# eigenfoo/littlemcmc

Measured on AMD Instinct MI355X. Metric: leapfrog-steps/sec (all chains), higher is better.
Workload: dtype f64

## Files before the change

### littlemcmc_amd/csrc/lmc_sampler.hpp

```cpp
#pragma once
#include "lmc_rng.hpp"
#include "lmc_targets.hpp"
#include "lmc_team.hpp"

namespace lmc {

constexpr int kStatusBadInitialEnergy = 1;

enum StatF64 : int {
    kSfStepSize = 0,
    kSfStepSizeBar = 1,
    kSfAccept = 2,
    kSfEnergyError = 3,
    kSfEnergy = 4,
    kSfMaxEnergyError = 5,
    kSfModelLogp = 6,
    kNumStatF64 = 7
};
enum StatI32 : int { kSiDepth = 0 , kSiTreeSize = 1 , kNumStatI32 = 2 };
enum StatU8 : int { kSbDiverging = 0, kSbTune = 1, kSbAccepted = 2, kNumStatU8 = 3 };
enum Counter : int { kCtMaxTreedepth = 0, kCtDivsSample = 1, kCtSamplesAfterTune = 2, kCtLeapfrogs = 3, kCtWaveTicks = 4, kNumCounters = 5 };

struct StatRecord {
    double f64[kNumStatF64];
// ... 377 lines not shown
        tm.sync();
        if (tm.wave() == 0) {
            rng_normals(r, d, out, stage);
            if (lane_id() == 0) {
                bcast[0] = static_cast<double>(r.pos);
                bcast[1] = static_cast<double>(r.has_gauss);
                bcast[2] = r.gauss;
            }
        }
        tm.sync();
        r.pos = first_i32(static_cast<int>(bcast[0]));
        r.has_gauss = first_i32(static_cast<int>(bcast[1]));
        r.gauss = first_f64(bcast[2]);
    }
}

template <int NS, class Target, class TeamT>
__device__ __forceinline__ void leapfrog(TeamT& tm, const Target& tgt, const double (&var)[NS], double eps,
                                         double (&q)[NS], double (&p)[NS], double (&g)[NS],
                                         double& energy, double& logp) {
    const double dt = 0.5 * eps;
#pragma unroll
    for (int s = 0; s < NS; ++s) {
        p[s] = p[s] + dt * g[s];
        const double v = var[s] * p[s];
        q[s] = q[s] + eps * v;
    }
    if constexpr (Target::kLanePartial) {
        double lp = tgt.logp_grad_partial(tm, q, g);
        double kin = 0.0;
#pragma unroll
        for (int s = 0; s < NS; ++s) {
            p[s] = p[s] + dt * g[s];
            kin = __builtin_fma(p[s], var[s] * p[s], kin);
        }
        tm.sum2(lp, kin);
        logp = lp;
        energy = 0.5 * kin - logp;
    } else {
        logp = first_f64(tgt.logp_grad(tm, q, g));
        double kin = 0.0;
#pragma unroll
        for (int s = 0; s < NS; ++s) {
            p[s] = p[s] + dt * g[s];
            kin = __builtin_fma(p[s], var[s] * p[s], kin);
        }
        energy = 0.5 * tm.sum(kin) - logp;
    }
}

typedef __attribute__((address_space(3))) double lds_double;
typedef __attribute__((address_space(1))) double glb_double;
template <int NS, class PTR>
__device__ __forceinline__ void vload_as(PTR base, double (&x)[NS]) {
    PTR p = base + LMC_CHAIN_THREAD * NS;
#pragma unroll
    for (int s = 0; s < NS; ++s) x[s] = p[s];
}
template <int NS, class PTR>
__device__ __forceinline__ void vstore_as(PTR base, const double (&x)[NS]) {
    PTR p = base + LMC_CHAIN_THREAD * NS;
#pragma unroll
    for (int s = 0; s < NS; ++s) p[s] = x[s];
}
struct LevelScalars {
    double w, a, pe, plogp;
    __device__ __forceinline__ void put(int j, double w_, double a_, double c, double d) {
        if (lane_id() == j) { w = w_; a = a_; pe = c; plogp = d; }
    }
    __device__ __forceinline__ void get(int j, double& w_, double& a_, double& c, double& d) const {
        w_ = readlane_f64(w, j); a_ = readlane_f64(a, j); c = readlane_f64(pe, j); d = readlane_f64(plogp, j);
    }
};

struct TransitionOut {
    double accept;
    double energy, energy_error, max_energy_error, model_logp;
    int depth;
    int n_leapfrog;
    int diverging;
    int exhausted;
    int accepted;
};

template <class P>
__device__ inline void hmc_transition_any(P& pol, double e0, double logp0, double step_size, double emax, double path_length,
                                          int max_steps, TransitionOut& out) {
    const double plen = first_f64(pol.uniform() * path_length);
    int n_steps = static_cast<int>(plen / step_size);
    n_steps = n_steps < 1 ? 1 : n_steps;
    n_steps = n_steps > max_steps ? max_steps : n_steps;
    typename P::End c;
    pol.start_state(c);
    double energy = e0, logp = logp0;
    for (int i = 0; i < n_steps; ++i) pol.leapfrog(step_size, c, energy, logp);
    bool diverging = !isfinite(energy);
    double de = first_f64(e0 - energy);
    if (isnan(de)) de = -__builtin_inf();
    if (fabs(de) > emax) diverging = true;
    const double accept = first_f64(fmin(1.0, exp_uniform(de)));
    bool accepted = false;
    if (!diverging) {
        const double u = pol.uniform();
        if (!(u >= accept)) { accepted = true; pol.accept_state(c); }
    }
    out.accept = accept;
    out.energy = energy;
    out.energy_error = de;
    out.max_energy_error = plen;
    out.model_logp = logp;
    out.depth = n_steps;
    out.n_leapfrog = n_steps;
    out.diverging = diverging;
    out.exhausted = 0;
    out.accepted = accepted;
}

template <int NS, class Target, class TeamT>
struct FusedHmcPolicy {
    static constexpr int kNS = NS;
    struct End { double q[NS], p[NS], g[NS]; };
    TeamT& tm; const Target& tgt; const double (&var)[NS]; RngState& rng;
    double (&q)[NS]; const double (&p0)[NS]; const double (&g0)[NS];
    UniformWindow win;
    __device__ __forceinline__ double uniform() { return team_uniform(tm, rng, win); }
    __device__ __forceinline__ void start_state(End& c) const { vcopy(c.q, q); vcopy(c.p, p0); vcopy(c.g, g0); }
    __device__ __forceinline__ void leapfrog(double eps, End& c, double& energy, double& logp) {
        lmc::leapfrog<NS>(tm, tgt, var, eps, c.q, c.p, c.g, energy, logp);
    }
    __device__ __forceinline__ void accept_state(const End& c) { vcopy(q, c.q); }
};
template <int NS, class Target, class TeamT>
__device__ inline void hmc_transition(TeamT& tm, const Target& tgt, const double (&var)[NS], RngState& rng,
                                      double (&q)[NS], const double (&p0)[NS], const double (&g0)[NS],
                                      double e0, double logp0, double step_size, double emax,
                                      double path_length, int max_steps, TransitionOut& out) {
    FusedHmcPolicy<NS, Target, TeamT> pol{tm, tgt, var, rng, q, p0, g0, UniformWindow{0.0, 0, 0}};
    hmc_transition_any(pol, e0, logp0, step_size, emax, path_length, max_steps, out);
}

#ifndef LMC_EXP_LANES_SLOAD
#define LMC_EXP_LANES_SLOAD 2
#endif
constexpr int kRedValues = 6;
constexpr int kExpTableDoubles = 32;
constexpr int kLevelScalDoubles = 96;
#ifndef LMC_PAIR_COLD_LDS
#define LMC_PAIR_COLD_LDS 3
#endif
enum ColdSlot : int { kColdAold = 0, kColdPsum = 1, kColdOp = 2, kColdOq = 3, kColdOg = 4, kNumCold = 5 };
constexpr int kNumColdSlots = kNumCold;

constexpr int run_leaf_group(int ns, int w) { return (w == 1 && ns <= 2) ? 4 : 2; }
template <int NS, int W = 1, int PL = 0, int G = 2>
struct PairLds {
    static_assert(G == 2 || (G == 4 && W == 1), "leaf quads exist for the one-wave kernels");
    static constexpr int DP = 64 * NS * W;
    static constexpr int kRedRows = G == 4 ? 8 : kRedValues;
    static constexpr int kRedWave = 64 * kRedRows;
    static constexpr int kRedSize = (2 * DP > W * kRedWave) ? 2 * DP : W * kRedWave;
    static constexpr int kExp = kRedSize;
    static constexpr int kXsum = kExp + kExpTableDoubles;
    static constexpr int kXsumSize = W > 1 ? 2 * 8 * W : 0;
    static constexpr int kScal = kXsum + kXsumSize;
    static constexpr int kCold = kScal + W * kLevelScalDoubles;
    static_assert(PL == 0 || W == 1, "the deep-tree plan exists for one-wave kernels");
    static constexpr int kColdLds = PL == 1 ? (NS >= 4 ? 0 : (LMC_PAIR_COLD_LDS < 1 ? LMC_PAIR_COLD_LDS : 1))
                                            : (W >= 8 ? (LMC_PAIR_COLD_LDS < 2 ? LMC_PAIR_COLD_LDS : 2) : LMC_PAIR_COLD_LDS);
    static constexpr int kQStage = (G == 4 && (NS >= 2 || PL == 0)) ? 2 : 0;
    static constexpr int kL1 = kCold + kColdLds * DP;
    static constexpr int kL2 = kL1 + (G == 4 ? kQStage : 3) * DP;
    static constexpr int kMinDoubles = kL2;
    static constexpr int kGlbLevels = (kNumCold - kColdLds) * DP;
    __host__ __device__ static constexpr int total_doubles(int nlds) { return kL2 + (nlds > 1 ? (nlds - 1) * 4 * DP : 0); }
};
#ifdef LMC_EXPERIMENTAL_SHAPES
#define LMC_PAIR_SHAPES(X) X(1, 1) X(2, 1) X(4, 1) X(4, 2) X(4, 4) X(2, 8) X(2, 2) X(1, 4)
#else
#define LMC_PAIR_SHAPES(X) X(1, 1) X(2, 1) X(4, 1) X(4, 2) X(4, 4)
#endif
constexpr int pair_min_doubles(int ns, int w, int plan = 0, int g = 2) {
#define X(NSV, WV) if (ns == NSV && w == WV) {                                                                               \
        if (g == 4 && run_leaf_group(NSV, WV) == 4)                                                                          \
            return plan == 1 ? PairLds<NSV, 1, 1, 4>::kMinDoubles : PairLds<NSV, 1, 0, 4>::kMinDoubles;                      \
        return (plan == 1 && WV == 1) ? PairLds<NSV, 1, 1>::kMinDoubles : PairLds<NSV, WV, 0>::kMinDoubles; }
    LMC_PAIR_SHAPES(X)
#undef X
    return 1 << 30;
}
constexpr int pair_total_doubles(int ns, int w, int nlds, int plan = 0, int g = 2) {
#define X(NSV, WV) if (ns == NSV && w == WV) {                                                                               \
        if (g == 4 && run_leaf_group(NSV, WV) == 4)                                                                          \
            return plan == 1 ? PairLds<NSV, 1, 1, 4>::total_doubles(nlds) : PairLds<NSV, 1, 0, 4>::total_doubles(nlds);      \
        return (plan == 1 && WV == 1) ? PairLds<NSV, 1, 1>::total_doubles(nlds) : PairLds<NSV, WV, 0>::total_doubles(nlds); }
    LMC_PAIR_SHAPES(X)
#undef X
    return 1 << 30;
}

struct PairCtx {
    double* lds;
    double* glb;
    int nlds;
    int red_lane;
    int wave_red;
    int wave_scal;
    int wave;
    int xpar;
};

template <int NS, int W = 1, int PL = 0, int G = 2>
__device__ __forceinline__ void red_put(const PairCtx& cx, int v, double x) {
    if constexpr (W == 1) ((lds_double*)cx.lds)[v * 64 + lane_id()] = x;
    else ((lds_double*)cx.lds)[v * 64 + lane_id() + cx.wave_red] = x;
}
template <int NS, int W = 1, int PL = 0, int G = 2>
__device__ __forceinline__ double red_gather(PairCtx& cx) {
    typedef double d2 __attribute__((ext_vector_type(2)));
    typedef __attribute__((address_space(3))) d2 lds_d2;
    asm volatile("" ::: "memory");
    unsigned r0 = static_cast<unsigned>(cx.red_lane);
    asm volatile("" : "+v"(r0));
    lds_double* L = (lds_double*)cx.lds;
    const d2 a = *(const lds_d2*)(size_t)(r0), b = *(const lds_d2*)(size_t)(r0 ^ 16u);
    const d2 c = *(const lds_d2*)(size_t)(r0 ^ 32u), d = *(const lds_d2*)(size_t)(r0 ^ 48u);
    asm volatile("" ::: "memory");
    double s = ((a.x + a.y) + (b.x + b.y)) + ((c.x + c.y) + (d.x + d.y));
    s += dpp_f64<0x111>(s);
    s += dpp_f64<0x112>(s);
    s += dpp_f64<0x114>(s);
    if constexpr (W > 1) {
        const int lane = lane_id();
        lds_double* xs = L + (PairLds<NS, W, PL, G>::kXsum + cx.xpar * (8 * W)) + (lane >> 3) * W;
        if ((lane & 7) == 7) xs[cx.wave] = s;
        __syncthreads();
        double t = xs[0];
#pragma unroll
        for (int w = 1; w < W; ++w) t += xs[w];
        s = t;
        cx.xpar ^= 1;
    }
    return s;
}
__device__ __forceinline__ int red_lane_init(int rows = kRedValues) {
    const int lane = lane_id();
    const int row = lane < 8 * rows ? lane : 0;
    return row * 8 + 2 * ((lane >> 2) & 3);
}
__device__ __forceinline__ bool red_any_nonpositive(double s, int k0, int n) {
    const unsigned long long m = ballot64(s <= 0.0);
    unsigned long long sel = 0ull;
    for (int k = k0; k < k0 + n; ++k) sel |= 1ull << (8 * k + 7);
    return (m & sel) != 0ull;
}

__constant__ double kExpLanesConst[8] = {46.166241308446828,
                                         2.16608493865351192654e-02,
                                         5.96317165397058656256e-12,
                                         1.0 / 720.0, 1.0 / 120.0, 1.0 / 24.0, 1.0 / 6.0, 0.0};
struct ExpLanesConst { double inv, hi, lo, c6, c5, c4, c3; };
__device__ __forceinline__ ExpLanesConst exp_lanes_const() {
    ExpLanesConst c;
#if LMC_EXP_LANES_SLOAD == 2
    typedef const __attribute__((address_space(4))) double cst_double;
    cst_double* p = (cst_double*)kExpLanesConst;
    asm volatile("" : "+s"(p));
    c.inv = p[0]; c.hi = p[1]; c.lo = p[2]; c.c6 = p[3]; c.c5 = p[4]; c.c4 = p[5]; c.c3 = p[6];
#elif LMC_EXP_LANES_SLOAD == 1
    c.inv = kExpLanesConst[0]; c.hi = kExpLanesConst[1]; c.lo = kExpLanesConst[2];
    c.c6 = kExpLanesConst[3]; c.c5 = kExpLanesConst[4]; c.c4 = kExpLanesConst[5]; c.c3 = kExpLanesConst[6];
#else
    c.inv = LMC_SC(46.166241308446828); c.hi = LMC_SC(2.16608493865351192654e-02); c.lo = LMC_SC(5.96317165397058656256e-12);
    c.c6 = LMC_SC(1.0 / 720.0); c.c5 = LMC_SC(1.0 / 120.0); c.c4 = LMC_SC(1.0 / 24.0); c.c3 = LMC_SC(1.0 / 6.0);
#endif
    return c;
}
template <int NS, int W = 1, int PL = 0, int G = 2>
__device__ __forceinline__ double exp_lanes(const PairCtx& cx, const ExpLanesConst& c, double x) {
    const double kf = rint(x * c.inv);
    double r = __builtin_fma(-kf, c.hi, x);
    r = __builtin_fma(-kf, c.lo, r);
    const int ki = static_cast<int>(kf);
    const double t = ((const lds_double*)cx.lds)[PairLds<NS, W, PL, G>::kExp + (ki & 31)];
    double p = fma_sgpr_addend(r, c.c6, c.c5);
    p = fma_sgpr_addend(p, r, c.c4);
    p = fma_sgpr_addend(p, r, c.c3);
    p = __builtin_fma(p, r, 0.5);
    p = __builtin_fma(p, r, 1.0);
    p = __builtin_fma(p, r, 1.0);
    return ldexp(p * t, ki >> 5);
}

template <int NS, int W, int PL, int G, int SLOT>
__device__ __forceinline__ void cold_load(const PairCtx& cx, double (&x)[NS]) {
    using L = PairLds<NS, W, PL, G>;
    if constexpr (SLOT < L::kColdLds) vload_as<NS>((lds_double*)cx.lds + (L::kCold + SLOT * L::DP), x);
    else vload_as<NS>((glb_double*)cx.glb + (SLOT - L::kColdLds) * L::DP, x);
}
template <int NS, int W, int PL, int G, int SLOT>
__device__ __forceinline__ void cold_store(const PairCtx& cx, const double (&x)[NS]) {
    using L = PairLds<NS, W, PL, G>;
    if constexpr (SLOT < L::kColdLds) vstore_as<NS>((lds_double*)cx.lds + (L::kCold + SLOT * L::DP), x);
    else vstore_as<NS>((glb_double*)cx.glb + (SLOT - L::kColdLds) * L::DP, x);
}
template <int NS, int W = 1, int PL = 0, int G = 2>
__device__ __forceinline__ void level1_load(const PairCtx& cx, double (&lp)[NS], double (&rp)[NS], double (&ps)[NS]) {
// ... 212 lines not shown
        int qsrc = -1;
        auto prop_q = [&](double (&t)[NS]) {
            if (qsrc == -1) vcopy(t, cq);
            else if (qsrc == -2) vcopy(t, eq);
            else if (G == 4 && qsrc < -2) {
                if constexpr (PairLds<NS, W, PL, G>::kQStage > 0)
                    vload_as<NS>((lds_double*)cx.lds + (PairLds<NS, W, PL, G>::kL1 + (qsrc == -3 ? PairLds<NS, W, PL, G>::DP : 0)), t);
                else if (qsrc == -3) vcopy(t, q1r);
                else vcopy(t, q0r);
            } else level_load_q<NS, W, PL, G>(cx, qsrc, t);
        };
        int elane = 15;
        double en_last = 0.0, lp_last = 0.0;
        const int D = depth;
        if (D == 0) {
            double v[NS], kinp, lp, en, ev;
            leapfrog_partial<NS>(tm, tgt, var, eps, cq, cp, cg, v, kinp, lp);
            red_put<NS, W, PL, G>(cx, 0, kinp); red_put<NS, W, PL, G>(cx, 1, lp);
            const double s0 = red_gather<NS, W, PL, G>(cx);
            if (leaf_scalars(s0, 1, en, ev) == 1) {
                tw = readlane_f64(ev, 15); ta = readlane_f64(ev, 14);
                en_last = en; lp_last = s0;
                vcopy(tps, cp);
            }
        } else if (G == 2 || D == 1) {
            const int n_pairs = 1 << (D - 1);
            for (int k = 0; k < n_pairs; ++k) {
                double v[NS], kinA, lpA, kinB, lpB;
                leapfrog_partial<NS>(tm, tgt, var, eps, cq, cp, cg, v, kinA, lpA);
                red_put<NS, W, PL, G>(cx, 0, kinA); red_put<NS, W, PL, G>(cx, 1, lpA);
                vcopy(eq, cq); vcopy(ep, cp);
                leapfrog_partial<NS>(tm, tgt, var, eps, cq, cp, cg, v, kinB, lpB);
                red_put<NS, W, PL, G>(cx, 2, kinB); red_put<NS, W, PL, G>(cx, 3, lpB);
#pragma unroll
                for (int s = 0; s < NS; ++s) tps[s] = ep[s] + cp[s];
                red_put<NS, W, PL, G>(cx, 4, pdot_v<NS>(tps, var, ep));
                red_put<NS, W, PL, G>(cx, 5, pdot<NS>(tps, v));
                const double s0 = red_gather<NS, W, PL, G>(cx);
                const int m = __builtin_ctz(~static_cast<unsigned>(k) | (1u << (D - 1)));
                double en, ev;
                if (leaf_scalars(s0, 2, en, ev) != 2) break;
                {
                    const double wA = readlane_f64(ev, 15), aA = readlane_f64(ev, 14);
                    const double wB = readlane_f64(ev, 31), aB = readlane_f64(ev, 30);
                    const bool turn = red_any_nonpositive(s0, 4, 2);
                    const double wsum = wA + wB;
                    const bool take_b = uniform_true(team_uniform(tm, rng, win) * wsum < wB);
                    qsrc = take_b ? -1 : -2;
                    elane = take_b ? 31 : 15;
                    en_last = en; lp_last = s0;
                    tw = wsum; ta = aA + aB;
                    if (turn) { turning = true; break; }
                }
                if constexpr (G == 2) {
                if (m >= 1) {
                    double alp[NS], arp[NS], aps[NS];
                    double aw, aa;
                    level1_load<NS, W, PL, G>(cx, alp, arp, aps);
                    level_scal_get_wa<NS, W, PL, G>(cx, 1, aw, aa);
                    const double sj = cascade_dots<NS, W, PL, G>(cx, var, alp, arp, aps, ep, tps, v);
                    const bool turn = red_any_nonpositive(sj, 0, 6);
                    const double wsum = aw + tw;
                    const bool take_b = uniform_true(team_uniform(tm, rng, win) * wsum < tw);
                    if (!take_b) qsrc = 1;
                    tw = wsum; ta = aa + ta;
                    if (turn) { turning = true; break; }
                }
                for (int j = 2; j <= m; ++j) {
                    double blp[NS], brp[NS], bps[NS], tl[NS];
                    levelN_load<NS, W, PL, G>(cx, j, 0, blp); levelN_load<NS, W, PL, G>(cx, j, 1, brp); levelN_load<NS, W, PL, G>(cx, j, 2, bps);
                    level_load_lp<NS, W, PL, G>(cx, j - 1, tl);
                    double bw, ba;
                    level_scal_get_wa<NS, W, PL, G>(cx, j, bw, ba);
                    const double sj = cascade_dots<NS, W, PL, G>(cx, var, blp, brp, bps, tl, tps, v);
                    const bool turn = red_any_nonpositive(sj, 0, 6);
                    const double wsum = bw + tw;
                    const bool take_b = uniform_true(team_uniform(tm, rng, win) * wsum < tw);
                    if (!take_b) qsrc = j;
                    tw = wsum; ta = ba + ta;
                    if (turn) { turning = true; break; }
                }
                if (turning) break;
                if (k + 1 < n_pairs) {
                    double tl[NS], tqv[NS];
                    if (m == 0) vcopy(tl, ep); else level_load_lp<NS, W, PL, G>(cx, m, tl);
                    if (qsrc == -1) vcopy(tqv, cq);
                    else if (qsrc == -2) vcopy(tqv, eq);
                    else level_load_q<NS, W, PL, G>(cx, qsrc, tqv);
#ifndef LMC_PARK_REORDER_MIN_NS
#define LMC_PARK_REORDER_MIN_NS 4
#endif
                    constexpr bool kParkReorder = NS >= LMC_PARK_REORDER_MIN_NS;
                    if constexpr (kParkReorder) level_scal_park<NS, W, PL, G>(cx, m + 1, tw, ta, qsrc, elane, en_last, lp_last);
                    if (m == 0) {
                        level1_store<NS, W, PL, G>(cx, tl, cp, tqv);
                    } else {
                        if constexpr (kParkReorder) {
#pragma unroll
                            for (int s = 0; s < NS; ++s) asm volatile("" : "+v"(tl[s]), "+v"(tqv[s]));
                        }
                        levelN_store<NS, W, PL, G>(cx, m + 1, 0, tl); levelN_store<NS, W, PL, G>(cx, m + 1, 1, cp);
                        levelN_store<NS, W, PL, G>(cx, m + 1, 2, tps); levelN_store<NS, W, PL, G>(cx, m + 1, 3, tqv);
                    }
                    if constexpr (!kParkReorder) level_scal_park<NS, W, PL, G>(cx, m + 1, tw, ta, qsrc, elane, en_last, lp_last);
                }
                }
            }
        } else if constexpr (G == 4) {
            using L = PairLds<NS, W, PL, G>;
            lds_double* const qst = (lds_double*)cx.lds + L::kL1;
            const int n_quads = 1 << (D - 2);
            for (int k = 0; k < n_quads; ++k) {
                static_assert(NS <= 2, "leaf quads: the left end of a depth-2 subtree waits in two rows of the reduction buffer");
                double v[NS], kin, lpl, a0[NS], a1[NS];
                leapfrog_partial<NS>(tm, tgt, var, eps, cq, cp, cg, v, kin, lpl);
                red_put<NS, W, PL, G>(cx, 0, kin); red_put<NS, W, PL, G>(cx, 1, lpl);
                if constexpr (L::kQStage > 0) vstore_as<NS>(qst, cq); else vcopy(q0r, cq);
                vcopy(a0, cp);
                leapfrog_partial<NS>(tm, tgt, var, eps, cq, cp, cg, v, kin, lpl);
                red_put<NS, W, PL, G>(cx, 2, kin); red_put<NS, W, PL, G>(cx, 3, lpl);
                if constexpr (L::kQStage > 0) vstore_as<NS>(qst + L::DP, cq); else vcopy(q1r, cq);
                vcopy(a1, cp);
                leapfrog_partial<NS>(tm, tgt, var, eps, cq, cp, cg, v, kin, lpl);
                red_put<NS, W, PL, G>(cx, 4, kin); red_put<NS, W, PL, G>(cx, 5, lpl);
                vcopy(eq, cq); vcopy(ep, cp);
                leapfrog_partial<NS>(tm, tgt, var, eps, cq, cp, cg, v, kin, lpl);
                red_put<NS, W, PL, G>(cx, 6, kin); red_put<NS, W, PL, G>(cx, 7, lpl);
                const double s0 = red_gather<NS, W, PL, G>(cx);
                double ta01[NS], va1[NS];
#pragma unroll
                for (int s = 0; s < NS; ++s) { ta01[s] = a0[s] + a1[s]; va1[s] = var[s] * a1[s]; tps[s] = ep[s] + cp[s]; }
                red_put<NS, W, PL, G>(cx, 0, pdot_v<NS>(ta01, var, a0));
                red_put<NS, W, PL, G>(cx, 1, pdot<NS>(ta01, va1));
                red_put<NS, W, PL, G>(cx, 2, pdot_v<NS>(tps, var, ep));
                red_put<NS, W, PL, G>(cx, 3, pdot<NS>(tps, v));
                double s1, s2;
                {
                    double d0 = 0.0, d1 = 0.0, d2 = 0.0, d3 = 0.0, d4 = 0.0, d5 = 0.0;
#pragma unroll
                    for (int s = 0; s < NS; ++s) {
                        const double p1 = ta01[s] + ep[s];
                        const double p2 = a1[s] + tps[s];
                        const double ps = ta01[s] + tps[s];
                        const double valp = var[s] * a0[s], vtlp = var[s] * ep[s], varp = var[s] * a1[s];
                        d0 = __builtin_fma(ps, valp, d0); d1 = __builtin_fma(ps, v[s], d1);
                        d2 = __builtin_fma(p1, valp, d2); d3 = __builtin_fma(p1, vtlp, d3);
                        d4 = __builtin_fma(p2, varp, d4); d5 = __builtin_fma(p2, v[s], d5);
                        tps[s] = ps;
                    }
                    red_put<NS, W, PL, G>(cx, 4, d0); red_put<NS, W, PL, G>(cx, 5, d1);
                    red_put<NS, W, PL, G>(cx, 6, d2); red_put<NS, W, PL, G>(cx, 7, d3);
                    s1 = red_gather<NS, W, PL, G>(cx);
                    red_put<NS, W, PL, G>(cx, 0, d4); red_put<NS, W, PL, G>(cx, 1, d5);
                    s2 = red_gather<NS, W, PL, G>(cx);
                }
                const unsigned long long np1 = ballot64(s1 <= 0.0), np2 = ballot64(s2 <= 0.0);
                const ExpLanesConst ec = exp_lanes_const();
                const double en = 0.5 * dpp_f64<0x118>(s0) - s0;
                double de_x = en - e0;
                const unsigned long long rare = ballot64(!(fabs(de_x) < emax)) | ballot64((-de_x) - coff > 600.0);
                de_x = isnan(de_x) ? __builtin_inf() : de_x;
                auto weights = [&]() {
                    const double x = -de_x;
                    const double xn = dpp_f64<0x101>(x);
                    const double arg = odd_lane ? (x - coff) : ((xn - coff) + fmin(xn, 0.0));
                    return exp_lanes<NS, W, PL, G>(cx, ec, arg);
                };
                double twA = 0.0, taA = 0.0;
                auto leaves_seq = [&](int i0, bool hold) -> int {
                    int seen = 0;
                    for (int i = i0; i < i0 + 2; ++i) {
                        const double dei = readlane_f64(de_x, 15 + 16 * i);
                        ++n_leap; ++seen;
                        if (!(fabs(dei) < emax)) { diverging = true; break; }
                        const double xi = -dei;
                        if (xi - coff > 600.0) {
                            const double f = exp_uniform(coff - xi);
                            const int lane = lane_id();
                            if (lane >= 1 && lane < kLevelScalDoubles / 4) {
                                lds_double* sc = (lds_double*)cx.lds + (L::kScal + 4 * lane);
                                sc[0] = sc[0] * f; sc[1] = sc[1] * f;
                            }
                            if (hold) { twA = twA * f; taA = taA * f; }
                            coff = xi;
                        }
                    }
                    return seen;
                };
                const bool fast = (rare & ((1ull << 15) | (1ull << 31) | (1ull << 47) | (1ull << 63))) == 0ull;
                auto mde_update = [&](double dx, bool examined) {
                    const bool upd = (fabs(dx) > fabs(mde)) & examined;
                    mde = upd ? dx : mde;
                };
                int seen = 2;
                if (fast) n_leap += 2; else seen = leaves_seq(0, false);
                double ev = weights();
                double w2 = readlane_f64(ev, 47), a2w = readlane_f64(ev, 46), w3 = readlane_f64(ev, 63), a3w = readlane_f64(ev, 62);
                mde_update(de_x, lane15 | (lane31 & (seen == 2)));
                if (diverging) break;
                int elane_a;
                {
                    const double w0 = readlane_f64(ev, 15), a0w = readlane_f64(ev, 14);
                    const double w1 = readlane_f64(ev, 31), a1w = readlane_f64(ev, 30);
                    const bool turn = (np1 & ((1ull << 7) | (1ull << 15))) != 0ull;
                    const double wsum = w0 + w1;
                    const bool take_b = uniform_true(team_uniform(tm, rng, win) * wsum < w1);
                    elane_a = take_b ? 31 : 15;
                    twA = wsum; taA = a0w + a1w;
                    if (turn) { turning = true; break; }
                }
                if (fast) n_leap += 2;
                else {
                    seen = leaves_seq(2, true);
                    ev = weights();
                    w2 = readlane_f64(ev, 47); a2w = readlane_f64(ev, 46); w3 = readlane_f64(ev, 63); a3w = readlane_f64(ev, 62);
                }
                mde_update(upper_half_down(de_x), lane15 | (lane31 & (seen == 2)));
                if (diverging) break;
                {
                    const bool turn = (np1 & ((1ull << 23) | (1ull << 31))) != 0ull;
                    const double wsum = w2 + w3;
                    const bool take_b = uniform_true(team_uniform(tm, rng, win) * wsum < w3);
                    elane = take_b ? 63 : 47;
                    tw = wsum; ta = a2w + a3w;
                    if (turn) { turning = true; break; }
                }
                {
                    const bool turn = ((np1 & ((1ull << 39) | (1ull << 47) | (1ull << 55) | (1ull << 63))) |
                                       (np2 & ((1ull << 7) | (1ull << 15)))) != 0ull;
                    const double wsum = twA + tw;
                    const bool take_b = uniform_true(team_uniform(tm, rng, win) * wsum < tw);
                    if (!take_b) elane = elane_a;
                    tw = wsum; ta = taA + ta;
                    qsrc = elane == 63 ? -1 : elane == 47 ? -2 : elane == 31 ? -3 : -4;
                    en_last = en; lp_last = s0;
                    if (turn) { turning = true; break; }
                }
                const int m = 1 + __builtin_ctz(~static_cast<unsigned>(k) | (1u << (D - 2)));
                for (int j = 2; j <= m; ++j) {
                    double blp[NS], brp[NS], bps[NS], tl[NS];
                    levelN_load<NS, W, PL, G>(cx, j, 0, blp); levelN_load<NS, W, PL, G>(cx, j, 1, brp); levelN_load<NS, W, PL, G>(cx, j, 2, bps);
                    if (j == 2) vcopy(tl, a0); else levelN_load<NS, W, PL, G>(cx, j - 1, 0, tl);
                    double bw, ba;
                    level_scal_get_wa<NS, W, PL, G>(cx, j, bw, ba);
                    const double sj = cascade_dots<NS, W, PL, G>(cx, var, blp, brp, bps, tl, tps, v);
                    const bool turn = red_any_nonpositive(sj, 0, 6);
                    const double wsum = bw + tw;
                    const bool take_b = uniform_true(team_uniform(tm, rng, win) * wsum < tw);
                    if (!take_b) qsrc = j;
                    tw = wsum; ta = ba + ta;
                    if (turn) { turning = true; break; }
                }
                if (turning) break;
                if (k + 1 < n_quads) {
                    double tl[NS], tqv[NS];
                    if (m == 1) vcopy(tl, a0); else levelN_load<NS, W, PL, G>(cx, m, 0, tl);
                    prop_q(tqv);
                    levelN_store<NS, W, PL, G>(cx, m + 1, 0, tl); levelN_store<NS, W, PL, G>(cx, m + 1, 1, cp);
                    levelN_store<NS, W, PL, G>(cx, m + 1, 2, tps); levelN_store<NS, W, PL, G>(cx, m + 1, 3, tqv);
                    level_scal_park<NS, W, PL, G>(cx, m + 1, tw, ta, qsrc, elane, en_last, lp_last);
                } else if (D == 2) {
#pragma unroll
                    for (int s = 0; s < NS; ++s) ((lds_double*)cx.lds)[(6 + s) * 64 + lane_id()] = a0[s];
                }
            }
        }
        ++depth;
        if (diverging || turning) { exhausted = false; break; }

        double wn = tot[0], an = tot[1], w_start = tot[2];
        const double c_tot = tot[3];
        if (uniform_true(c_tot != coff)) {
            const double f = exp_uniform(first_f64(c_tot) - coff);
            wn = wn * f; an = an * f; w_start = w_start * f;
            if (lane_id() == 0) { tot[2] = w_start; tot[3] = coff; }
        }
        if (uniform_true(team_uniform(tm, rng, win) * (w_start + wn) < tw)) {
            double tqv[NS];
            prop_q(tqv);
            vstore_as<NS>((glb_double*)qrow, tqv);
            if (qsrc < 0) {
                prop_e = readlane_f64(en_last, elane); prop_logp = readlane_f64(lp_last, elane);
            } else {
                double w_, a_;
                level_scal_get<NS, W, PL, G>(cx, qsrc, w_, a_, prop_e, prop_logp);
                prop_e = first_f64(prop_e); prop_logp = first_f64(prop_logp);
            }
        }
        if (lane_id() == 0) { tot[0] = wn + tw; tot[1] = an + ta; }
        double tlp[NS], psum[NS], op[NS], aold[NS];
        if (D == 0) vcopy(tlp, cp);
        else if (D == 1) vcopy(tlp, ep);
        else if (G == 4 && D == 2) {
#pragma unroll
            for (int s = 0; s < NS; ++s) tlp[s] = ((const lds_double*)cx.lds)[(6 + s) * 64 + lane_id()];
        }
        else level_load_lp<NS, W, PL, G>(cx, D - 1, tlp);
        cold_load<NS, W, PL, G, kColdPsum>(cx, psum); cold_load<NS, W, PL, G, kColdOp>(cx, op); cold_load<NS, W, PL, G, kColdAold>(cx, aold);
#pragma unroll
        for (int s = 0; s < NS; ++s) {
            const double t = psum[s] + tps[s];
            psum[s] = momentum_f32 ? static_cast<double>(static_cast<float>(t)) : t;
        }
        cold_store<NS, W, PL, G, kColdPsum>(cx, psum);
        double ov[NS], av[NS];
        end_velocity<NS>(ov, var, op, o_start);
        end_velocity<NS>(av, var, aold, aold_start);
        double d0 = 0.0, d1 = 0.0, d2 = 0.0, d3 = 0.0, d4 = 0.0, d5 = 0.0;
        if (right) {
#pragma unroll
            for (int s = 0; s < NS; ++s) {
                const double vtl = var[s] * tlp[s], vtr = var[s] * cp[s];
                const double p1 = psum[s] + tlp[s], p2 = aold[s] + tps[s];
                d0 = __builtin_fma(psum[s], ov[s], d0); d1 = __builtin_fma(psum[s], vtr, d1);
                d2 = __builtin_fma(p1, ov[s], d2);      d3 = __builtin_fma(p1, vtl, d3);
                d4 = __builtin_fma(p2, av[s], d4);      d5 = __builtin_fma(p2, vtr, d5);
            }
        } else {
#pragma unroll
            for (int s = 0; s < NS; ++s) {
                const double vtl = var[s] * tlp[s], vtr = var[s] * cp[s];
                const double p1 = tps[s] + aold[s], p2 = tlp[s] + psum[s];
                d0 = __builtin_fma(psum[s], vtr, d0);   d1 = __builtin_fma(psum[s], ov[s], d1);
                d2 = __builtin_fma(p1, vtr, d2);        d3 = __builtin_fma(p1, av[s], d3);
                d4 = __builtin_fma(p2, vtl, d4);        d5 = __builtin_fma(p2, ov[s], d5);
            }
        }
        c_start = false;
        red_put<NS, W, PL, G>(cx, 0, d0); red_put<NS, W, PL, G>(cx, 1, d1); red_put<NS, W, PL, G>(cx, 2, d2);
        red_put<NS, W, PL, G>(cx, 3, d3); red_put<NS, W, PL, G>(cx, 4, d4); red_put<NS, W, PL, G>(cx, 5, d5);
        if (red_any_nonpositive(red_gather<NS, W, PL, G>(cx), 0, 6)) { turning = true; exhausted = false; break; }
    }

    const double wn_end = first_f64(tot[0]), an_end = first_f64(tot[1]);
    const double mean_accept = (wn_end > 0.0) ? first_f64(an_end / wn_end) : 0.0;
    out.accept = mean_accept;
    out.energy = prop_e;
    out.energy_error = first_f64(prop_e - e0);
    out.max_energy_error = mde_combined();
    out.model_logp = prop_logp;
    out.depth = depth;
    out.n_leapfrog = n_leap;
    out.diverging = diverging;
    out.exhausted = exhausted;
    out.accepted = 0;
}

#ifndef LMC_NORMALS_IN_REGS
#define LMC_NORMALS_IN_REGS 1
#endif
#ifndef LMC_WAVES_NS1
#define LMC_WAVES_NS1 4
#endif
#ifndef LMC_WAVES_NS2
#define LMC_WAVES_NS2 3
#endif
#ifndef LMC_WAVES_NS4
#define LMC_WAVES_NS4 2
#endif
#ifndef LMC_WAVES_NS2_W8
#define LMC_WAVES_NS2_W8 4
#endif
constexpr int run_waves_per_simd(int ns, int w = 1) {
    return (ns == 2 && w == 8) ? LMC_WAVES_NS2_W8 : ns <= 1 ? LMC_WAVES_NS1 : ns == 2 ? LMC_WAVES_NS2 : ns == 4 ? LMC_WAVES_NS4 : 1;
}
constexpr int kLdsMtDoubles = 320;
#ifndef LMC_MT_IN_LDS_W1
#define LMC_MT_IN_LDS_W1 1
#endif
constexpr bool run_mt_in_lds(int w) { return w > 1 || LMC_MT_IN_LDS_W1; }
constexpr int lds_tail_doubles(int w) {
    return w == 1 ? (run_mt_in_lds(1) ? kLdsMtDoubles : 0) : kLdsMtDoubles + 2 * w * kTeamSlots + 4 + (w >= 4 ? kLdsMtDoubles : 0);
}
constexpr int kPlanUp = 24, kPlanDown = 14;

template <class CA, class PT>
__device__ __forceinline__ int stop_request_load(const CA& A, const PT& P, int chain_in_launch, int it, long long git, long long leaps = -1) {
    int* dev = A.stop_dev;
    const int mask = P.relay_mask;
    const bool relay = (it == 0) ? ((chain_in_launch & mask) == 0)
                                 : ((git & 15) == 0 && ((chain_in_launch + static_cast<int>(git >> 4)) & mask) == 0);
    if (relay) {
        if (__hip_atomic_load(A.stop, __ATOMIC_RELAXED, __HIP_MEMORY_SCOPE_SYSTEM) != 0)
            __hip_atomic_store(dev, 1, __ATOMIC_RELAXED, __HIP_MEMORY_SCOPE_AGENT);
        __hip_atomic_store(A.progress, static_cast<int>(git), __ATOMIC_RELAXED, __HIP_MEMORY_SCOPE_SYSTEM);
        if (leaps >= 0 && it >= 8 && A.tree_hint != nullptr) {
            int mean = static_cast<int>(static_cast<float>(leaps) / static_cast<float>(it));
            mean = mean < 1 ? 1 : (mean > 4095 ? 4095 : mean);
            const int at = git > 0x7ffff ? 0x7ffff : static_cast<int>(git);
            __hip_atomic_store(A.tree_hint, (at << 12) | mean, __ATOMIC_RELAXED, __HIP_MEMORY_SCOPE_SYSTEM);
        }
    }
    return __hip_atomic_load(dev, __ATOMIC_RELAXED, __HIP_MEMORY_SCOPE_AGENT);
}
template <class TeamT>
__device__ __forceinline__ bool stop_requested(TeamT& tm, int loaded, double* bcast) {
    if constexpr (TeamT::kWaves == 1) {
        return first_i32(loaded) != 0;
    } else {
// ... 405 lines not shown
```

Measured before the change: 3.435 billion.

## Merge leaf-quad multinomial picks across lanes and fold level-2 turn dots into reduction

On the fast path, the per-quad multinomial merges (pair A, pair B, then AB) are computed together with lane-parallel swap-adds and ballots. This replaces three sequential team_uniform draws and readlanes, and the window and RNG positions are advanced explicitly. For odd quads, the level-2 U-turn dot products are also computed in the same reduction gather as s2, which removes the separate cascade_dots reduction at j==2. This adds complexity in RNG-state bookkeeping and some extra LDS loads on odd quads.

```diff
diff --git a/littlemcmc_amd/csrc/lmc_sampler.hpp b/littlemcmc_amd/csrc/lmc_sampler.hpp
--- a/littlemcmc_amd/csrc/lmc_sampler.hpp
+++ b/littlemcmc_amd/csrc/lmc_sampler.hpp
@@ -553,6 +553,9 @@
 constexpr int kNumColdSlots = kNumCold;
 
 constexpr int run_leaf_group(int ns, int w) { return (w == 1 && ns <= 2) ? 4 : 2; }
+#ifndef LMC_QUAD_LANE_MERGES
+#define LMC_QUAD_LANE_MERGES 1
+#endif
 template <int NS, int W = 1, int PL = 0, int G = 2>
 struct PairLds {
     static_assert(G == 2 || (G == 4 && W == 1), "leaf quads exist for the one-wave kernels");
@@ -1071,8 +1074,26 @@
                     red_put<NS, W, PL, G>(cx, 6, d2); red_put<NS, W, PL, G>(cx, 7, d3);
                     s1 = red_gather<NS, W, PL, G>(cx);
                     red_put<NS, W, PL, G>(cx, 0, d4); red_put<NS, W, PL, G>(cx, 1, d5);
-                    s2 = red_gather<NS, W, PL, G>(cx);
                 }
+                if (k & 1) {
+                    double blp[NS], brp[NS], bps[NS];
+                    levelN_load<NS, W, PL, G>(cx, 2, 0, blp); levelN_load<NS, W, PL, G>(cx, 2, 1, brp); levelN_load<NS, W, PL, G>(cx, 2, 2, bps);
+                    double d0 = 0.0, d1 = 0.0, d2 = 0.0, d3 = 0.0, d4 = 0.0, d5 = 0.0;
+#pragma unroll
+                    for (int s = 0; s < NS; ++s) {
+                        const double p1 = bps[s] + a0[s];
+                        const double p2 = brp[s] + tps[s];
+                        const double ps = bps[s] + tps[s];
+                        const double valp = var[s] * blp[s], vtlp = var[s] * a0[s], varp = var[s] * brp[s];
+                        d0 = __builtin_fma(ps, valp, d0); d1 = __builtin_fma(ps, v[s], d1);
+                        d2 = __builtin_fma(p1, valp, d2); d3 = __builtin_fma(p1, vtlp, d3);
+                        d4 = __builtin_fma(p2, varp, d4); d5 = __builtin_fma(p2, v[s], d5);
+                        tps[s] = ps;
+                    }
+                    red_put<NS, W, PL, G>(cx, 2, d0); red_put<NS, W, PL, G>(cx, 3, d1); red_put<NS, W, PL, G>(cx, 4, d2);
+                    red_put<NS, W, PL, G>(cx, 5, d3); red_put<NS, W, PL, G>(cx, 6, d4); red_put<NS, W, PL, G>(cx, 7, d5);
+                }
+                s2 = red_gather<NS, W, PL, G>(cx);
                 const unsigned long long np1 = ballot64(s1 <= 0.0), np2 = ballot64(s2 <= 0.0);
                 const ExpLanesConst ec = exp_lanes_const();
                 const double en = 0.5 * dpp_f64<0x118>(s0) - s0;
@@ -1111,59 +1132,93 @@
                     const bool upd = (fabs(dx) > fabs(mde)) & examined;
                     mde = upd ? dx : mde;
                 };
-                int seen = 2;
-                if (fast) n_leap += 2; else seen = leaves_seq(0, false);
-                double ev = weights();
-                double w2 = readlane_f64(ev, 47), a2w = readlane_f64(ev, 46), w3 = readlane_f64(ev, 63), a3w = readlane_f64(ev, 62);
-                mde_update(de_x, lane15 | (lane31 & (seen == 2)));
-                if (diverging) break;
-                int elane_a;
-                {
-                    const double w0 = readlane_f64(ev, 15), a0w = readlane_f64(ev, 14);
-                    const double w1 = readlane_f64(ev, 31), a1w = readlane_f64(ev, 30);
-                    const bool turn = (np1 & ((1ull << 7) | (1ull << 15))) != 0ull;
-                    const double wsum = w0 + w1;
-                    const bool take_b = uniform_true(team_uniform(tm, rng, win) * wsum < w1);
-                    elane_a = take_b ? 31 : 15;
-                    twA = wsum; taA = a0w + a1w;
-                    if (turn) { turning = true; break; }
-                }
-                if (fast) n_leap += 2;
-                else {
-                    seen = leaves_seq(2, true);
-                    ev = weights();
-                    w2 = readlane_f64(ev, 47); a2w = readlane_f64(ev, 46); w3 = readlane_f64(ev, 63); a3w = readlane_f64(ev, 62);
-                }
-                mde_update(upper_half_down(de_x), lane15 | (lane31 & (seen == 2)));
-                if (diverging) break;
-                {
-                    const bool turn = (np1 & ((1ull << 23) | (1ull << 31))) != 0ull;
-                    const double wsum = w2 + w3;
-                    const bool take_b = uniform_true(team_uniform(tm, rng, win) * wsum < w3);
-                    elane = take_b ? 63 : 47;
-                    tw = wsum; ta = a2w + a3w;
-                    if (turn) { turning = true; break; }
-                }
-                {
-                    const bool turn = ((np1 & ((1ull << 39) | (1ull << 47) | (1ull << 55) | (1ull << 63))) |
-                                       (np2 & ((1ull << 7) | (1ull << 15)))) != 0ull;
-                    const double wsum = twA + tw;
-                    const bool take_b = uniform_true(team_uniform(tm, rng, win) * wsum < tw);
-                    if (!take_b) elane = elane_a;
-                    tw = wsum; ta = taA + ta;
+                if (LMC_QUAD_LANE_MERGES && fast && first_i32(win.n) - first_i32(win.idx) >= 3) {
+                    n_leap += 2;
+                    const double ev = weights();
+                    mde_update(de_x, lane15 | lane31);
+                    const double y = swap16_add(ev, ev);
+                    const double z = swap32_add(y, y);
+                    const int i0 = first_i32(win.idx);
+                    const double uA = readlane_f64(win.val, i0), uB = readlane_f64(win.val, i0 + 1), uAB = readlane_f64(win.val, i0 + 2);
+                    const unsigned long long take = (ballot64(uA * y < ev) & (1ull << 31)) |
+                                                    (ballot64(uB * y < ev) & (1ull << 63));
+                    const bool take_ab = (ballot64(uAB * z < y) & (1ull << 63)) != 0ull;
+                    const bool turn_a = (np1 & ((1ull << 7) | (1ull << 15))) != 0ull;
+                    const bool turn_b = (np1 & ((1ull << 23) | (1ull << 31))) != 0ull;
+                    const bool turn_ab = ((np1 & ((1ull << 39) | (1ull << 47) | (1ull << 55) | (1ull << 63))) |
+                                          (np2 & ((1ull << 7) | (1ull << 15)))) != 0ull;
+                    const int used = turn_a ? 1 : turn_b ? 2 : 3;
+                    win.idx = i0 + used;
+                    rng.pos = first_i32(rng.pos) + 2 * used;
+                    if (turn_a) { turning = true; break; }
+                    n_leap += 2;
+                    mde_update(upper_half_down(de_x), lane15 | lane31);
+                    if (turn_b) { turning = true; break; }
+                    elane = take_ab ? ((take & (1ull << 63)) ? 63 : 47) : ((take & (1ull << 31)) ? 31 : 15);
+                    tw = readlane_f64(z, 63); ta = readlane_f64(z, 62);
                     qsrc = elane == 63 ? -1 : elane == 47 ? -2 : elane == 31 ? -3 : -4;
                     en_last = en; lp_last = s0;
-                    if (turn) { turning = true; break; }
+                    if (turn_ab) { turning = true; break; }
+                } else {
+                    int seen = 2;
+                    if (fast) n_leap += 2; else seen = leaves_seq(0, false);
+                    double ev = weights();
+                    double w2 = readlane_f64(ev, 47), a2w = readlane_f64(ev, 46), w3 = readlane_f64(ev, 63), a3w = readlane_f64(ev, 62);
+                    mde_update(de_x, lane15 | (lane31 & (seen == 2)));
+                    if (diverging) break;
+                    int elane_a;
+                    {
+                        const double w0 = readlane_f64(ev, 15), a0w = readlane_f64(ev, 14);
+                        const double w1 = readlane_f64(ev, 31), a1w = readlane_f64(ev, 30);
+                        const bool turn = (np1 & ((1ull << 7) | (1ull << 15))) != 0ull;
+                        const double wsum = w0 + w1;
+                        const bool take_b = uniform_true(team_uniform(tm, rng, win) * wsum < w1);
+                        elane_a = take_b ? 31 : 15;
+                        twA = wsum; taA = a0w + a1w;
+                        if (turn) { turning = true; break; }
+                    }
+                    if (fast) n_leap += 2;
+                    else {
+                        seen = leaves_seq(2, true);
+                        ev = weights();
+                        w2 = readlane_f64(ev, 47); a2w = readlane_f64(ev, 46); w3 = readlane_f64(ev, 63); a3w = readlane_f64(ev, 62);
+                    }
+                    mde_update(upper_half_down(de_x), lane15 | (lane31 & (seen == 2)));
+                    if (diverging) break;
+                    {
+                        const bool turn = (np1 & ((1ull << 23) | (1ull << 31))) != 0ull;
+                        const double wsum = w2 + w3;
+                        const bool take_b = uniform_true(team_uniform(tm, rng, win) * wsum < w3);
+                        elane = take_b ? 63 : 47;
+                        tw = wsum; ta = a2w + a3w;
+                        if (turn) { turning = true; break; }
+                    }
+                    {
+                        const bool turn = ((np1 & ((1ull << 39) | (1ull << 47) | (1ull << 55) | (1ull << 63))) |
+                                           (np2 & ((1ull << 7) | (1ull << 15)))) != 0ull;
+                        const double wsum = twA + tw;
+                        const bool take_b = uniform_true(team_uniform(tm, rng, win) * wsum < tw);
+                        if (!take_b) elane = elane_a;
+                        tw = wsum; ta = taA + ta;
+                        qsrc = elane == 63 ? -1 : elane == 47 ? -2 : elane == 31 ? -3 : -4;
+                        en_last = en; lp_last = s0;
+                        if (turn) { turning = true; break; }
+                    }
                 }
                 const int m = 1 + __builtin_ctz(~static_cast<unsigned>(k) | (1u << (D - 2)));
                 for (int j = 2; j <= m; ++j) {
-                    double blp[NS], brp[NS], bps[NS], tl[NS];
-                    levelN_load<NS, W, PL, G>(cx, j, 0, blp); levelN_load<NS, W, PL, G>(cx, j, 1, brp); levelN_load<NS, W, PL, G>(cx, j, 2, bps);
-                    if (j == 2) vcopy(tl, a0); else levelN_load<NS, W, PL, G>(cx, j - 1, 0, tl);
+                    bool turn;
+                    if (j == 2) {
+                        turn = (np2 & ((1ull << 23) | (1ull << 31) | (1ull << 39) | (1ull << 47) | (1ull << 55) | (1ull << 63))) != 0ull;
+                    } else {
+                        double blp[NS], brp[NS], bps[NS], tl[NS];
+                        levelN_load<NS, W, PL, G>(cx, j, 0, blp); levelN_load<NS, W, PL, G>(cx, j, 1, brp); levelN_load<NS, W, PL, G>(cx, j, 2, bps);
+                        levelN_load<NS, W, PL, G>(cx, j - 1, 0, tl);
+                        const double sj = cascade_dots<NS, W, PL, G>(cx, var, blp, brp, bps, tl, tps, v);
+                        turn = red_any_nonpositive(sj, 0, 6);
+                    }
                     double bw, ba;
                     level_scal_get_wa<NS, W, PL, G>(cx, j, bw, ba);
-                    const double sj = cascade_dots<NS, W, PL, G>(cx, var, blp, brp, bps, tl, tps, v);
-                    const bool turn = red_any_nonpositive(sj, 0, 6);
                     const double wsum = bw + tw;
                     const bool take_b = uniform_true(team_uniform(tm, rng, win) * wsum < tw);
                     if (!take_b) qsrc = j;
```

Measured after the change: 3.454 billion (median of 6 runs). About the same (+0.6%).
